# nianticlabs/acezero

Hardware: AMD Instinct MI355X
Metric: ACE patches/sec (higher is better)
Workload: dtype bf16; 1 GPU; 7-Scenes-chess-like ace_zero mapping step: 8M-patch bf16 feature buffer in HBM, batch 5120 per GPU, default head (1 block, 2 103 300 params), tanh loss, 1cyclepoly AdamW, pose_refinement none; buffer_patches=8000000, batch_per_gpu=5120, global_batch=5120, parallelism=dp1

## Files before the change

acezero_amd/_native.py:

```python
import contextlib
import ctypes as C
import os

import torch

from . import build as _build

_lib = None

ACEZ_OK = 0
ERRORS = {-1: "ACEZ_ERR_INVALID", -2: "ACEZ_ERR_HIP", -3: "ACEZ_ERR_NODEVICE", -4: "ACEZ_ERR_NAN"}


class RansacParams(C.Structure):
    _fields_ = [("hypotheses", C.c_int32), ("max_tries", C.c_int32), ("inlier_threshold", C.c_float),
                ("inlier_alpha", C.c_float), ("max_reproj", C.c_float), ("subsampling", C.c_int32),
                ("max_ref_steps", C.c_int32), ("reserved", C.c_int32)]


class Intrinsics(C.Structure):
    _fields_ = [("focal", C.c_float), ("ppx", C.c_float), ("ppy", C.c_float)]


class HeadDesc(C.Structure):
# ... 106 lines not shown
    "acez_trainer_create": (C.c_int, [C.POINTER(C.c_void_p), C.POINTER(TrainConfig), C.POINTER(ParamBuffers), C.c_int]),
    "acez_trainer_destroy": (None, [C.c_void_p]),
    "acez_trainer_set_buffer": (C.c_int, [C.c_void_p, C.POINTER(TrainBuffer)]),
    "acez_trainer_sync_weights": (C.c_int, [C.c_void_p, C.c_void_p]),
    "acez_train_backward": (C.c_int, [C.c_void_p, C.c_void_p, C.c_int, C.c_void_p]),
    "acez_train_update": (C.c_int, [C.c_void_p, C.c_void_p]),
    "acez_train_update_next": (C.c_int, [C.c_void_p, C.c_void_p, C.c_int, C.c_void_p]),
    "acez_train_update_layers": (C.c_int, [C.c_void_p, C.c_int, C.c_int, C.c_void_p]),
    "acez_trainer_export_weights16": (C.c_int, [C.c_void_p, C.c_int, C.c_int, C.c_void_p, C.c_void_p]),
    "acez_trainer_import_weights16": (C.c_int, [C.c_void_p, C.c_int, C.c_int, C.c_void_p, C.c_void_p]),
    "acez_trainer_import_weights16_all": (C.c_int, [C.c_void_p, C.c_int, C.c_int, C.c_void_p, C.c_void_p]),
    "acez_train_step": (C.c_int, [C.c_void_p, C.c_void_p, C.c_int, C.c_void_p]),
    "acez_train_step_next": (C.c_int, [C.c_void_p, C.c_void_p, C.c_int, C.c_void_p, C.c_int, C.c_void_p]),
    "acez_train_group_create": (C.c_int, [C.POINTER(C.c_void_p), C.POINTER(C.c_void_p), C.c_int]),
    "acez_train_group_destroy": (None, [C.c_void_p]),
    "acez_train_group_step": (C.c_int, [C.c_void_p, C.POINTER(C.c_void_p), C.POINTER(C.c_int32), C.POINTER(C.c_void_p),
                                        C.POINTER(C.c_int32), C.c_void_p]),
    "acez_trainer_get_state": (C.c_int, [C.c_void_p, C.POINTER(TrainState), C.c_void_p]),
    "acez_trainer_get_log": (C.c_int, [C.c_void_p, C.c_int, C.c_int, C.c_void_p, C.c_void_p, C.c_void_p]),
    "acez_trainer_last_scene_coords": (C.c_int, [C.c_void_p, C.c_void_p, C.c_int, C.c_void_p]),
    "acez_trainer_set_profiling": (C.c_int, [C.c_void_p, C.c_int]),
    "acez_trainer_get_profile": (C.c_int, [C.c_void_p, C.c_void_p, C.c_void_p]),
    "acez_trainer_seq_status": (C.c_int, [C.c_void_p, C.POINTER(C.c_int), C.POINTER(C.c_int), C.POINTER(C.c_int)]),
    "acez_trainer_debug_read": (C.c_int, [C.c_void_p, C.c_int, C.c_int, C.c_void_p, C.c_int64, C.c_void_p]),
    "acez_trainer_get_poses": (C.c_int, [C.c_void_p, C.c_void_p, C.c_void_p]),
    "acez_head_forward": (C.c_int, [C.c_void_p, C.c_void_p, C.c_int, C.c_void_p, C.c_void_p]),
    "acez_head_forward_maps": (C.c_int, [C.c_void_p, C.c_void_p, C.c_int, C.c_int, C.c_int, C.c_void_p, C.c_void_p]),
    "acez_buffer_warp_views": (C.c_int, [C.c_void_p, C.c_int, C.c_int, C.c_int, C.c_void_p, C.c_void_p, C.c_void_p, C.c_int, C.c_int, C.c_int,
                                        C.c_void_p, C.c_void_p, C.c_int, C.c_int, C.c_void_p, C.c_void_p]),
    "acez_buffer_sample_views": (C.c_int, [C.c_void_p, C.c_void_p, C.c_int, C.c_int, C.c_int, C.c_int, C.c_int, C.c_uint64, C.c_uint64,
                                           C.c_int32, C.c_void_p, C.c_void_p, C.c_void_p, C.c_void_p, C.c_void_p]),
    "acez_buffer_sample_views_table": (C.c_int, [C.c_void_p, C.c_int64, C.c_void_p, C.c_int64, C.c_void_p, C.c_int, C.c_int, C.c_int, C.c_int,
                                                 C.c_uint64, C.c_uint64, C.c_int32, C.c_void_p, C.c_void_p, C.c_void_p, C.c_void_p,
                                                 C.c_void_p]),
    "acez_encoder_create": (C.c_int, [C.POINTER(C.c_void_p), C.POINTER(C.c_void_p), C.POINTER(C.c_void_p), C.c_int, C.c_int, C.c_int,
                                      C.c_int, C.c_int, C.c_int]),
    "acez_encoder_destroy": (None, [C.c_void_p]),
    "acez_encoder_output_size": (C.c_int, [C.c_int, C.c_int, C.POINTER(C.c_int), C.POINTER(C.c_int)]),
    "acez_encoder_forward": (C.c_int, [C.c_void_p, C.c_void_p, C.c_int, C.c_int, C.c_int, C.c_void_p, C.c_void_p]),
    "acez_point_cloud_filter": (C.c_int, [C.c_void_p, C.c_void_p, C.c_void_p, C.c_int, C.c_int, C.c_int, C.c_float, C.c_int, C.c_int,
                                          C.c_int, C.c_uint64, C.c_uint64, C.c_int, C.c_void_p, C.c_void_p, C.c_void_p, C.c_void_p,
                                          C.c_void_p, C.c_void_p]),
    "acez_align_create": (C.c_int, [C.POINTER(C.c_void_p), C.c_int, C.c_int, C.c_int]),
    "acez_align_destroy": (None, [C.c_void_p]),
    "acez_align_evaluate": (C.c_int, [C.c_void_p, C.c_void_p, C.c_void_p, C.c_void_p, C.c_int, C.POINTER(AlignParams), C.c_void_p,
                                      C.c_void_p, C.POINTER(C.c_double), C.POINTER(C.c_int32), C.c_void_p, C.c_void_p, C.c_void_p,
# ... 86 lines not shown
```

acezero_amd/csrc/head_api.hip:

```cpp
#include "head_kernels.hip"
#include "pose_fused.hip"
#include "head_maps.hip"
#include "acez_common.h"
#include "conv_launch.h"
#include <stdlib.h>
#include <string.h>
#include <algorithm>
#include "acez_common.h"
#include <vector>
#include <new>

using namespace acez;

struct StepCarry {
  bool wave_pending = false;
  const int64_t* idx = nullptr;
  int n = 0;
  bool in_alt = false;
  void hold(const int64_t* i, int k, bool alt) { idx = i; n = k; in_alt = alt; }
  void drop_batch() { hold(nullptr, 0, false); }
};

struct acez_trainer {
  char* arena_base = nullptr;
// ... 44 lines not shown
  bool pose_fused = true;
  int pose_tile = 4;
  bool pose_wt_valid = false;
  float* row_dT = nullptr;
  int* row_image = nullptr;
  bool profiling = false;
  std::vector<hipEvent_t> ev_pool;
  struct EvUse { int cls, i0, i1, launches; };
  std::vector<EvUse> ev_used;
  size_t ev_next = 0;
  int prof_launches = 0;
  bool seq = true;
  bool f16 = false;
  int last_nblk = 0;
  int n_cus = 0;
  uint32_t* seq_flags = nullptr;
  uint32_t seq_base[64] = {};
  uint32_t* seq_xcc = nullptr;
  int* seq_err = nullptr;
  uint32_t seq_spin_limit = 40000;
  int seq_faults = 0;
  int seq_probe = -1;
  bool loss_in_chain = true;
  long seq_launches = 0, seq_fault_at = -1;
  bool wgrad_opt = true;
  float* wg_xch = nullptr;
  uint32_t* wg_flags = nullptr;
  uint32_t wg_epoch = 0;
  uint16_t* R0_alt = nullptr;
  int4* batch_meta_alt = nullptr;
  long wgo_fault_at = -1;
  int wgo_fault_mod = 0;
  uint32_t* wg_status = nullptr;
  WgoFaultRec* wg_rec = nullptr;
  int wgo_recovered = 0;
  bool inference_only = false;
  bool sizing = false;
  size_t sized_total = 0;
  unsigned long long* pose_trace = nullptr;
  unsigned long long* wgo_trace = nullptr;
};

enum { KC_SCHED = 0, KC_GATHER, KC_GEMM_FWD, KC_LOSS, KC_GEMM_DGRAD, KC_WGRAD, KC_REDUCE, KC_ADAMW, KC_COUNT };

static int loss_blocks(int n) { return (n + 15) / 16; }
static int gather_blocks(int n) { return (n + 3) / 4 < 1024 ? (n + 3) / 4 : 1024; }
// ... 522 lines not shown
  a.In[f1] = tr->R[tr->nb + 1]; a.In[f2] = tr->out[f1];
  a.slabs = tr->slabs; a.slab_stride = tr->n_wide; a.M = n; a.nslabs = tr->nslabs; a.n_layers = tr->L; a.st = st; a.zeros = tr->zeros;
}


enum class Flow { Fused, Backward, Update };
enum class Opt { None, WgradOpt, AdamwPose, AdamwNext, AdamwSplitPose, Adamw };
enum class NextAt { None, Loss, Optimiser };

struct StepPlan {
  Flow flow;
  bool begin_launch = false, begin_gathers = false, begin_pose = false;
  NextAt next_at = NextAt::None;
  Opt opt = Opt::None;
};

struct StepRun {
  acez_trainer* tr;
  StepPlan plan;
  const int64_t* idx; int n;
  const int64_t* next; int n_next;
  int nblk;
  bool loss_in_chain = false;
  hipStream_t s, ps;
  const TrainState* st;
};

static StepPlan plan_step(const acez_trainer* tr, Flow flow, const int64_t* idx, int n, const int64_t* next, int n_next) {
  StepPlan p{flow};
  const bool pf = tr->pose_fused, announced = next && n_next > 0;
  if (flow != Flow::Update) {
    const StepCarry& c = tr->carry;
    const bool have = !c.in_alt && c.idx == idx && c.n == n;
    p.begin_gathers = !have || (!pf && c.wave_pending);
    p.begin_pose = pf;
    p.begin_launch = p.begin_gathers || pf;
    if (flow == Flow::Backward) return p;
  }
  if (flow == Flow::Fused && wgrad_opt_usable(tr)) p.opt = Opt::WgradOpt;
  else if (flow == Flow::Fused && pf) p.opt = Opt::AdamwPose;
  else if (announced && tr->cfg.pose_refinement == 0 && tr->have_buf) p.opt = Opt::AdamwNext;
  else if (tr->cfg.pose_refinement != 0) p.opt = Opt::AdamwSplitPose;
  else p.opt = Opt::Adamw;
  if (announced && (p.opt == Opt::WgradOpt || p.opt == Opt::AdamwPose)) p.next_at = NextAt::Loss;
  else if (p.opt == Opt::AdamwNext || (announced && p.opt == Opt::AdamwSplitPose && pf && tr->have_buf)) p.next_at = NextAt::Optimiser;
  return p;
// ... 103 lines not shown
    ++tr->prof_launches;
  };
  ProfScope dchain(tr, s, collect ? -1 : KC_GEMM_DGRAD);
  dgrad(f2, f1, nullptr, tr->dZ[f1], nullptr);
  int cur = 0;
  dgrad(f1, 3 * tr->nb + 2, nullptr, tr->dZ[3 * tr->nb + 2], tr->dR[cur]);
  for (int b = tr->nb; b >= 0; --b) {
    dgrad(3 * b + 2, 3 * b + 1, nullptr, tr->dZ[3 * b + 1], nullptr);
    dgrad(3 * b + 1, 3 * b, nullptr, tr->dZ[3 * b], nullptr);
    if (b > 0) {
      dgrad(3 * b, 3 * (b - 1) + 2, tr->dR[cur], tr->dZ[3 * (b - 1) + 2], tr->dR[cur ^ 1]);
      cur ^= 1;
    }
  }
  if (collect) *collect = sq;
  else if (seq && inchain) {
    const SeqLossArgs x = train_loss_in_chain(*inchain);
    launch_rowseq<true>(tr, sq, n, st, s, &x);
  }
  else if (seq) launch_rowseq<true>(tr, sq, n, st, s);
  else if (inchain) abort();
}

static void launch_weight_grads(acez_trainer* tr, const StepPlan& p, int n, int nblk, const TrainState* st, hipStream_t s) {
  const bool fused = p.flow == Flow::Fused;
  const int f2 = 3 * (tr->nb + 1) + 1;
  {
    GradReduceArgs a{};
    a.slabs = tr->slabs; a.slab_stride = tr->n_wide; a.nslabs = tr->nslabs; a.fc3_partials = tr->fc3_partials;
    a.fc3_stride = tr->fc3_stride; a.stat_partials = tr->stat_partials; a.n_loss_blocks = nblk; a.grad = tr->pb.d_grad;
    a.n_wide = tr->n_wide; a.n_params = tr->n_params; a.st = st;
    a.bias_partials = tr->bias_partials; a.bias_layer_stride = tr->bias_layer_stride; a.n_layers = tr->L;
    a.skip_wide = fused ? 1 : 0;
    a.fault = tr->seq_err;
    for (int l = 0; l < tr->L; ++l) a.bias_count[l] = (l == f2) ? nblk : (n + 79) / 80;
    tr->last_reduce = a;
  }
  {
    WgradArgs a{};
    fill_wgrad_args(tr, a, n, st);
    ProfScope ps(tr, s, KC_WGRAD);
    const int groups = tr->L * tr->nslabs;
    if (p.opt == Opt::WgradOpt) {
      WgradOptArgs o{};
      fill_adam_args(tr, o.ad);
      o.ad.tail = tr->last_reduce;
// ... 86 lines not shown
}

static void pose_fwd_launches(acez_trainer* tr, hipStream_t q) {
  if (tr->cfg.pose_refinement == 2) pose_forward(tr, &tr->st->active, q);
  if (tr->cfg.pose_refinement == 1)
    hipLaunchKernelGGL(pose_compose_kernel, dim3((tr->buf.n_images + 255) / 256), dim3(256), 0, q, (const float*)tr->pa1,
                       (const float*)tr->pb.d_pose_params, 1.0f, tr->pose_cur, tr->buf.n_images, (const int*)&tr->st->active, tr->cfg.pose_refinement_ortho);
}
static void pose_bwd_launches(acez_trainer* tr, int n, hipStream_t q) {
  if (tr->cfg.pose_refinement == 0) return;
  const int I = tr->buf.n_images;
  const int* active = &tr->st->active;
  hipLaunchKernelGGL(pose_grad_reduce2_kernel, dim3((I + 15) / 16), dim3(256), 0, q, (const float*)tr->row_dT, (const int*)tr->row_image, n, tr->pdT, I, active);
  if (tr->cfg.pose_refinement == 2) {
    hipLaunchKernelGGL(pose_mlp_bwd_kernel, dim3((I + PN_IMG - 1) / PN_IMG), dim3(256), 0, q, pose_net_args(tr, active));
    launch_pose_wgrad(tr, active, false, q);
  } else {
    hipLaunchKernelGGL(pose_compose_bwd_kernel, dim3((I + 255) / 256), dim3(256), 0, q, (const float*)tr->pa1, (const float*)tr->pb.d_pose_params, 1.0f,
                       (const float*)tr->pdT, tr->pb.d_grad + tr->n_params + 4, I, active, tr->cfg.pose_refinement_ortho);
  }
}

static StepRun start_run(acez_trainer* tr, Flow flow, const int64_t* idx, int n, const int64_t* next, int n_next, hipStream_t s) {
  return StepRun{tr, plan_step(tr, flow, idx, n, next, n_next), idx, n, next, n_next, loss_blocks(n), false, s, tr->pose_stream ? tr->pose_stream : s, nullptr};
}

static void launch_chain(const StepRun& r, bool bwd) {
  if (bwd) launch_dgrad(r.tr, r.n, r.st, r.s, nullptr, r.loss_in_chain ? &r : nullptr);
  else launch_forward(r.tr, r.tr->R[0], r.n, r.st, r.s);
}

template <class Chains>
static int run_steps(StepRun* runs, int count, Chains chains) {
  for (int i = 0; i < count; ++i) {
    StepRun& r = runs[i];
    acez_trainer* tr = r.tr;
    tr->last_n = r.n;
    begin_step(tr, r.plan, r.idx, r.n, r.s);
    r.st = tr->st;
    if (r.ps != r.s) {
      ACEZ_HIP_CHECK(hipEventRecord(tr->ev_begin, r.s));
      ACEZ_HIP_CHECK(hipStreamWaitEvent(r.ps, tr->ev_begin, 0));
    }
    if (!tr->pose_fused) pose_fwd_launches(tr, r.ps);
    if (r.ps != r.s) ACEZ_HIP_CHECK(hipEventRecord(tr->ev_pose_fwd, r.ps));
  }
  chains(false);
  for (int i = 0; i < count; ++i) {
    StepRun& r = runs[i];
    acez_trainer* tr = r.tr;
    if (r.ps != r.s) ACEZ_HIP_CHECK(hipStreamWaitEvent(r.s, tr->ev_pose_fwd, 0));
// ... 9 lines not shown
  for (int i = 0; i < count; ++i) {
    StepRun& r = runs[i];
    acez_trainer* tr = r.tr;
    launch_weight_grads(tr, r.plan, r.n, r.nblk, r.st, r.s);
    if (r.ps != r.s) ACEZ_HIP_CHECK(hipStreamWaitEvent(r.s, tr->ev_pose_bwd, 0));
    if (tr->pose_fused && r.plan.flow == Flow::Backward) launch_pose_wgrad(tr, &tr->st->active, false, r.s);
    ACEZ_HIP_CHECK(hipGetLastError());
    if (r.plan.flow == Flow::Fused) {
      const int rc = launch_update(tr, r.plan, r.s, 0, tr->L, r.next, r.n_next);
      if (rc != ACEZ_OK) return rc;
    }
  }
  return ACEZ_OK;
}

static int train_step_impl(acez_trainer* tr, Flow flow, const int64_t* d_indices, int n, void* stream, const int64_t* d_next = nullptr, int n_next = 0) {
  ACEZ_REQUIRE(tr && d_indices, "null pointer");
  ACEZ_REQUIRE(!tr->inference_only, "an inference-only context (acez_train_config.inference_only) cannot train");
  ACEZ_REQUIRE(tr->have_buf, "acez_trainer_set_buffer has not been called");
  ACEZ_REQUIRE(n > 0 && n <= tr->max_batch, "n must be in [1, max_batch]");
  ACEZ_HIP_CHECK(hipSetDevice(tr->device));
  StepRun r = start_run(tr, flow, d_indices, n, d_next, n_next, (hipStream_t)stream);
  r.loss_in_chain = tr->loss_in_chain && r.plan.opt == Opt::WgradOpt && seq_usable(tr, n);
  return run_steps(&r, 1, [&](bool bwd) { launch_chain(r, bwd); });
}

extern "C" int acez_train_backward(acez_trainer* tr, const int64_t* d_indices, int n, void* stream) {
  return train_step_impl(tr, Flow::Backward, d_indices, n, stream);
}

static int train_update_impl(acez_trainer* tr, void* stream, int layer_lo, int layer_hi, const int64_t* d_next = nullptr, int n_next = 0) {
  ACEZ_REQUIRE(tr, "null trainer");
  ACEZ_REQUIRE(!tr->inference_only, "an inference-only context (acez_train_config.inference_only) cannot train");
  if (layer_hi < 0) layer_hi = tr->L;
  ACEZ_REQUIRE(layer_lo >= 0 && layer_lo <= layer_hi && layer_hi <= tr->L, "layer range out of bounds");
  ACEZ_HIP_CHECK(hipSetDevice(tr->device));
  return launch_update(tr, plan_step(tr, Flow::Update, nullptr, 0, d_next, n_next), (hipStream_t)stream, layer_lo, layer_hi, d_next, n_next);
}

extern "C" int acez_train_update(acez_trainer* tr, void* stream) { return train_update_impl(tr, stream, 0, -1); }
extern "C" int acez_train_update_next(acez_trainer* tr, const int64_t* d_indices_next, int n_next, void* stream) {
  ACEZ_REQUIRE(n_next >= 0 && (!tr || n_next <= tr->max_batch), "n_next must be in [0, max_batch]");
  return train_update_impl(tr, stream, 0, -1, d_indices_next, n_next);
}

extern "C" int acez_train_update_layers(acez_trainer* tr, int layer_lo, int layer_hi, void* stream) {
  return train_update_impl(tr, stream, layer_lo, layer_hi);
// ... 239 lines not shown
```

acezero_amd/csrc/head_kernels.hip:

```cpp
#include <hip/hip_runtime.h>
#include <stdint.h>
#include "head_kernels.h"
#include "gemm_common.h"

namespace acez {


template <int GR = 4>
__device__ __forceinline__ void gather_rows(const uint16_t* __restrict__ feat, const int64_t* __restrict__ idx, uint16_t* __restrict__ out, int n,
                                            int wave, int nwaves, int lane, const GatherMeta& meta) {
  const bool held = meta.hold && *meta.hold;
  for (int r0 = wave; r0 < n; r0 += GR * nwaves) {
    int r[GR];
    bool ok[GR];
    int64_t s[GR];
#pragma unroll
    for (int j = 0; j < GR; ++j) { r[j] = r0 + j * nwaves; ok[j] = r[j] < n; s[j] = idx[ok[j] ? r[j] : r0]; }
    uint4 v[GR];
#pragma unroll
    for (int j = 0; j < GR; ++j) v[j] = *reinterpret_cast<const uint4*>(feat + s[j] * 512 + lane * 8);
    int view[GR];
    float2 tp[GR];
    if (meta.dst) {
#pragma unroll
// ... 390 lines not shown
}

struct SeqLayer {
  const uint16_t *In, *W;
  const float* bias;
  const uint16_t *add, *res;
  uint2* mask_out;
  const uint2* mask_in;
  uint16_t *out_main, *out_aux;
  float* bias_partials;
  int aux_mode, pad;
};
constexpr int SEQ_MAX_LAYERS = 8;
struct RowSeqArgs {
  SeqLayer layer[SEQ_MAX_LAYERS];
  int n_layers, M;
  const TrainState* st;
  uint32_t* flags;
  uint32_t base[64];
  uint32_t spin_limit;
  uint32_t* xcc_dbg;
};

template <bool BWD, class E, int SEAM0>
__device__ __forceinline__ void rowseq_layers(const RowSeqArgs& a, uint16_t* smem, const int mt, const int n0) {
  for (int layer = 0; layer < a.n_layers; ++layer) {
    const SeqLayer& y = a.layer[layer];
    RowGemmArgs g;
    g.In = y.In; g.W = y.W; g.bias = y.bias; g.add = y.add; g.mask_out = y.mask_out; g.mask_in = y.mask_in; g.res = y.res; g.out_main = y.out_main; g.out_aux = y.out_aux;
    g.bias_partials = y.bias_partials; g.M = a.M; g.N = 512; g.K = 512; g.relu = BWD ? 0 : 1; g.aux_mode = y.aux_mode; g.st = a.st;
    g.absmax = (BWD && a.st) ? const_cast<uint32_t*>(a.st->dz_absmax_slots) : nullptr;
    SeqLink q;
    q.flag = a.flags + mt * 32; q.target = (a.base[mt] + (uint32_t)(layer + SEAM0)) * 32u;
    q.first = !SEAM0 && layer == 0; q.wait = SEAM0 || layer > 0; q.signal = layer + 1 < a.n_layers;
    q.next_W = q.signal ? a.layer[layer + 1].W : nullptr;
    q.flag_index = (uint32_t)(mt * 32); q.limit = a.spin_limit;
    if (!BWD) {
      if (y.aux_mode == AUX_RESIDUAL) rowgemm80_body<true, false, false, AUX_RESIDUAL, true, E>(g, smem, 1, mt, n0, q);
      else rowgemm80_body<true, false, false, AUX_NONE, true, E>(g, smem, 1, mt, n0, q);
    } else {
      if (y.add) rowgemm80_body<false, true, true, AUX_UNMASKED, true, E>(g, smem, 1, mt, n0, q);
      else if (y.aux_mode == AUX_UNMASKED) rowgemm80_body<false, false, true, AUX_UNMASKED, true, E>(g, smem, 1, mt, n0, q);
      else rowgemm80_body<false, false, true, AUX_NONE, true, E>(g, smem, 1, mt, n0, q);
    }
  }
}

template <bool BWD, class E = EltBf16>
__global__ __launch_bounds__(512) void rowseq_kernel(RowSeqArgs a) {
  __shared__ __attribute__((aligned(16))) uint16_t smem[RG80_SMEM_SEQ];
  const int mtiles = (a.M + 79) / 80;
  const int per_xcd = (mtiles + 7) >> 3;
  const int jx = blockIdx.x >> 3;
  const int mt = (blockIdx.x & 7) * per_xcd + (jx >> 2);
  if (mt >= mtiles) return;
  if (a.xcc_dbg && threadIdx.x == 0) {
    const uint32_t xcc = __builtin_amdgcn_s_getreg((3 << 11) | 20) & 15u;
    atomicOr(a.xcc_dbg + (blockIdx.x & 7), 1u << xcc);
    a.xcc_dbg[8 + mt * 4 + (jx & 3)] = xcc;
  }
  if ((a.st && !a.st->active) || a.flags[64 * 32]) {
    if (threadIdx.x == 0) {
      const uint32_t inc = 8u * (uint32_t)(a.n_layers - 1);
      asm volatile("global_atomic_add %0, %1, off" ::"v"(a.flags + mt * 32), "v"(inc) : "memory");
    }
    return;
  }
  rowseq_layers<BWD, E, 0>(a, smem, mt, (jx & 3) * 128);
}

__global__ __launch_bounds__(512) void seq_probe_kernel(uint32_t* rec , int mtiles) {
  __shared__ __attribute__((aligned(16))) uint16_t smem[RG80_SMEM_SEQ];
  const int per_xcd = (mtiles + 7) >> 3;
  const int jx = blockIdx.x >> 3;
  const int mt = (blockIdx.x & 7) * per_xcd + (jx >> 2);
  if (threadIdx.x == 0) smem[0] = (uint16_t)blockIdx.x;
  __syncthreads();
  if (mt >= mtiles || threadIdx.x != 0) return;
  const uint32_t xcc = __builtin_amdgcn_s_getreg((3 << 11) | 20) & 15u;
  rec[mt * 4 + (jx & 3)] = (xcc << 16) | smem[0];
}

static inline void launch_rowgemm(const RowGemmArgs& g, hipStream_t s, bool f16 = false) {
  const bool br = g.bias != nullptr;
  const int mtiles = (g.M + 79) / 80;
  const dim3 grid(8 * 4 * ((mtiles + 7) / 8));
#define ACEZ_RG(...)                                                                                               \
  do {                                                                                                             \
    if (f16) hipLaunchKernelGGL((rowgemm80_kernel<__VA_ARGS__, EltF16>), grid, dim3(512), 0, s, g);                \
    else hipLaunchKernelGGL((rowgemm80_kernel<__VA_ARGS__>), grid, dim3(512), 0, s, g);                            \
  } while (0)
// ... 1253 lines not shown
  return -sum;
}

constexpr int WGO_PF = 17;
__device__ __forceinline__ void lds_wait_ge(uint32_t* f, uint32_t target) {
  while (__hip_atomic_load(f, __ATOMIC_RELAXED, __HIP_MEMORY_SCOPE_WORKGROUP) < target) __builtin_amdgcn_s_sleep(1);
  asm volatile("" ::: "memory");
}
__device__ __forceinline__ void lds_bump(uint32_t* f) {
  asm volatile("s_waitcnt lgkmcnt(0)" ::: "memory");
  if ((threadIdx.x & 63) == 0) __hip_atomic_fetch_add(f, 1u, __ATOMIC_RELAXED, __HIP_MEMORY_SCOPE_WORKGROUP);
}

struct SeqLossArgs {
  LossArgs loss;
  int nblk;
  const uint16_t* feat;
  const int64_t* idx_next;
  uint16_t* out_next;
  int n_next;
  GatherMeta meta;
};

template <class E = EltBf16>
__global__ __launch_bounds__(512) void rowseq_loss_kernel(RowSeqArgs a, SeqLossArgs x) {
  __shared__ __attribute__((aligned(16))) uint16_t smem[RG80_SMEM_SEQ];
  const int mtiles = (a.M + 79) / 80;
  const int per_xcd = (mtiles + 7) >> 3;
  const int jx = blockIdx.x >> 3;
  const int mt = (blockIdx.x & 7) * per_xcd + (jx >> 2);
  if (mt >= mtiles) return;
  const int t = threadIdx.x, l = t & 63;
  const int w = __builtin_amdgcn_readfirstlane(t >> 6);
  const int nt = jx & 3, n0 = nt * 128;
  if (a.xcc_dbg && t == 0) {
    const uint32_t xcc = __builtin_amdgcn_s_getreg((3 << 11) | 20) & 15u;
    atomicOr(a.xcc_dbg + (blockIdx.x & 7), 1u << xcc);
    a.xcc_dbg[8 + mt * 4 + nt] = xcc;
  }
  uint32_t* const qsync = reinterpret_cast<uint32_t*>(smem + RG80_SMEM);
  if (t < 2) qsync[t] = 0u;
  asm volatile("s_waitcnt lgkmcnt(0)" ::: "memory");
  __builtin_amdgcn_s_barrier();
  const bool dead = (a.st && !a.st->active) || a.flags[64 * 32];
  if (w >= 4) {
    const int lw = w - 4;
    if (!dead) {
#pragma unroll
      for (int j = 0; j < 4; ++j) {
        const int row = (lw * 4 + j) * 8 + (l >> 3);
        const uint16_t* g = a.layer[0].W + (size_t)(n0 + row) * 512 + ((l & 7) ^ ((row >> 1) & 7)) * 8;
#pragma unroll
        for (int kt = 0; kt < 4; ++kt)
          __builtin_amdgcn_global_load_lds((gvoid_t*)(g + kt * 64), (lvoid_t*)(smem + kt * RG80_STAGE + (lw * 4 + j) * 8 * 64), 16, 0, 0);
      }
    }
    if (nt != 0 && x.n_next > 0) gather_rows<8>(x.feat, x.idx_next, x.out_next, x.n_next, (mt * 3 + nt - 1) * 4 + lw, mtiles * 12, l, x.meta);
  }
  if (dead) {
    if (t == 0) {
      const uint32_t inc = 8u * (uint32_t)a.n_layers;
      asm volatile("global_atomic_add %0, %1, off" ::"v"(a.flags + mt * 32), "v"(inc) : "memory");
    }
    return;
  }
  if (w < 4 || nt == 0) {
    const int quartet = w >> 2;
    const int block = 5 * mt + (nt == 0 ? quartet : nt + 1);
    if (block < x.nblk) {
      float* scratch = reinterpret_cast<float*>(smem + 4 * RG80_STAGE) + quartet * (3 * 4 * 4 * 4);
      uint32_t* const f = qsync + quartet;
      loss_body<false, true, E, 4>(x.loss, block, w & 3, l, nullptr, scratch, LossPre{0, 0, 0, 0.f, 0.f}, [f] { lds_bump(f); lds_wait_ge(f, 4u); });
    }
    ACEZ_VMCNT(0);
    if (l == 0) {
      const uint32_t inc = nt == 0 ? 1u : 2u;
      asm volatile("global_atomic_add %0, %1, off" ::"v"(a.flags + mt * 32), "v"(inc) : "memory");
    }
  }
  rowseq_layers<true, E, 1>(a, smem, mt, n0);
}

#ifdef ACEZ_DIAG
#define WGO_STAMP(i) do { if (o.trace && (threadIdx.x & 63) == 0) o.trace[((size_t)blockIdx.x * 12 + (threadIdx.x >> 6)) * 8 + (i)] = __builtin_amdgcn_s_memtime(); } while (0)
#else
#define WGO_STAMP(i) do { } while (0)
#endif
template <class E = EltBf16>
__global__ __launch_bounds__(WGRAD_THREADS) void wgrad_opt_kernel(WgradArgs a, WgradOptArgs o, PostArgs post) {
  constexpr int RING = WGRAD_RING;
  static_assert(RING >= 3, "two free ring slots are used as staging areas after the K loop");
  __shared__ __attribute__((aligned(16))) uint16_t smem[RING][2][64 * 128];
  __shared__ uint32_t wsync[2];
  const int t = threadIdx.x, l = t & 63;
  const int w = __builtin_amdgcn_readfirstlane(t >> 6);
  const int b = blockIdx.x;
  const int xcd = b & 7, jx = b >> 3;
  const int layer = xcd + 8 * (jx >> 5), slab = (jx >> 4) & 1, tile = jx & 15;
  if (layer >= a.n_layers) return;
  if (t < 2) wsync[t] = 0;
  WGO_STAMP(0);
  const int n0 = (tile >> 2) * 128, c0 = (tile & 3) * 128;
  const AdamArgs& ad = o.ad;
// ... 234 lines not shown
```

acezero_amd/head.py:

```python
import ctypes as C
import math

import numpy as np
import torch

from . import DEFAULT_DTYPE
from . import _native as N

LOSS_TYPES = {"tanh": 0, "dyntanh": 1, "l1": 2, "l1+sqrt": 3, "l1+logl1": 4, "l1+log": 4}
SCHEDULES = {"constant": 0, "1cyclepoly": 1, "circle": 2}
DTYPES = {"bf16": 0, "fp16": 1}


def resolve_dtype(dtype=None):
    import os
    dtype = (dtype or os.environ.get("ACEZ_DTYPE") or DEFAULT_DTYPE).lower()
    if dtype in ("fp32", "float32"):
        raise NotImplementedError("fp32 arithmetic (--use_half False) is not implemented; choose dtype='fp16' (the reference's "
                                  "autocast format) or 'bf16'")
    if dtype not in DTYPES:
        raise ValueError("dtype must be 'bf16' or 'fp16'")
    return dtype


# ... 112 lines not shown
        cfg.max_batch, cfg.global_batch = self.max_batch, self.global_batch
        cfg.loss_type = LOSS_TYPES[loss_type]
        cfg.soft_clamp, cfg.soft_clamp_min, cfg.circle_schedule = soft_clamp, soft_clamp_min, int(circle_schedule)
        cfg.hard_clamp, cfg.depth_min, cfg.depth_max, cfg.depth_target = hard_clamp, depth_min, depth_max, depth_target
        cfg.inlier_px_threshold = inlier_px_threshold
        cfg.schedule, cfg.iterations = SCHEDULES[schedule], int(iterations)
        cfg.lr_min, cfg.lr_max, cfg.warmup_iterations, cfg.warmup_lr = lr_min, lr_max, int(warmup_iterations), warmup_lr
        cfg.cooldown_iterations, cfg.cooldown_trigger_percent = int(cooldown_iterations), cooldown_trigger_percent
        cfg.beta1, cfg.beta2, cfg.eps, cfg.weight_decay = 0.9, 0.999, 1e-8, 1e-2
        cfg.refine_calibration, cfg.focal_init, cfg.calib_lr = int(refine_calibration), float(focal_init), calib_lr
        cfg.pose_refinement = 2 if self.pose_mlp else (1 if self.pose_naive else 0)
        cfg.pose_refinement_wait, cfg.pose_refinement_lr = int(pose_refinement_wait), float(pose_refinement_lr)
        cfg.pose_refinement_weight = float(pose_refinement_weight)
        if refinement_ortho not in ("gram-schmidt", "procrustes"):
            raise ValueError("refinement_ortho must be 'gram-schmidt' or 'procrustes'")
        cfg.pose_refinement_ortho = 1 if refinement_ortho == "procrustes" else 0
        cfg.compute_dtype = DTYPES[self.dtype]
        cfg.inference_only = 1 if inference_only else 0
        pb = N.ParamBuffers(_ptr(self.params), _ptr(self.adam_m), _ptr(self.adam_v), _ptr(self.grad), self.n_params,
                            _ptr(self.pose_params), _ptr(self.pose_m), _ptr(self.pose_v), self.n_pose)
        h = C.c_void_p()
        N.check(self.lib.acez_trainer_create(C.byref(h), C.byref(cfg), C.byref(pb), self.device.index))
        self._h = h
        self._buf = None
        self.iterations = int(iterations)

    def close(self):
        if getattr(self, "_h", None):
            self.lib.acez_trainer_destroy(self._h)
            self._h = None

    def __del__(self):
        try:
            self.close()
        except Exception:
            pass

    def _views(self):
        out, o = {}, 0
        for name in layer_names(self.nb):
            out[name + ".weight"] = self.params[o:o + 262144].view(512, 512, 1, 1)
            o += 262144
            out[name + ".bias"] = self.params[o:o + 512]
            o += 512
        out["fc3.weight"] = self.params[o:o + self.no * 512].view(self.no, 512, 1, 1)
        o += self.no * 512
# ... 91 lines not shown

    def master_tensors(self):
        return [self.params, self.adam_m, self.adam_v]

    def step(self, indices, next_indices=None):
        assert indices.dtype == torch.int64 and indices.is_cuda and indices.is_contiguous()
        if next_indices is None:
            N.check(self.lib.acez_train_step(self._h, _ptr(indices), int(indices.numel()), _stream()))
        else:
            assert next_indices.dtype == torch.int64 and next_indices.is_cuda and next_indices.is_contiguous()
            self._next_keepalive = next_indices
            N.check(self.lib.acez_train_step_next(self._h, _ptr(indices), int(indices.numel()), _ptr(next_indices), int(next_indices.numel()),
                                                  _stream()))

    def state(self):
        st = N.TrainState()
        rc = self.lib.acez_trainer_get_state(self._h, C.byref(st), _stream())
        if rc not in (0, -4):
            N.check(rc)
        return {"iteration": st.iteration, "max_iterations": st.max_iterations, "in_cooldown": bool(st.in_cooldown),
                "nan": bool(st.nan_flag), "lr": st.lr, "loss": st.last_loss, "batch_inliers": st.last_batch_inliers,
                "focal_scale": st.focal_scale, "grad_scale": st.grad_scale, "opt_steps": st.opt_steps}

    def seq_status(self):
        en, pr, fl = C.c_int(0), C.c_int(0), C.c_int(0)
        N.check(self.lib.acez_trainer_seq_status(self._h, C.byref(en), C.byref(pr), C.byref(fl)))
        return {"enabled": bool(en.value), "probe": pr.value, "faults": fl.value}

    def log(self, first, count):
        loss = np.zeros(count, np.float32)
        inl = np.zeros(count, np.float32)
        N.check(self.lib.acez_trainer_get_log(self._h, first, count, loss.ctypes.data_as(C.c_void_p),
                                              inl.ctypes.data_as(C.c_void_p), _stream()))
        return loss, inl

    def last_scene_coords(self, n):
        out = np.zeros((n, 3), np.float32)
        N.check(self.lib.acez_trainer_last_scene_coords(self._h, out.ctypes.data_as(C.c_void_p), n, _stream()))
        return out

    KERNEL_CLASSES = ("sched", "gather", "gemm_fwd", "loss", "gemm_dgrad", "wgrad", "grad_reduce", "adamw")

    def set_profiling(self, on):
        N.check(self.lib.acez_trainer_set_profiling(self._h, int(bool(on))))

    def get_profile(self):
        ms = np.zeros(8, np.float32)
        cnt = np.zeros(8, np.int32)
        N.check(self.lib.acez_trainer_get_profile(self._h, ms.ctypes.data_as(C.c_void_p), cnt.ctypes.data_as(C.c_void_p)))
        return {k: (float(ms[i]), int(cnt[i])) for i, k in enumerate(self.KERNEL_CLASSES)}
# ... 82 lines not shown
```

include/acez.h:

```cpp
#ifndef ACEZ_H
#define ACEZ_H

#include <stdint.h>

#ifdef __cplusplus
extern "C" {
#endif

#define ACEZ_OK 0
#define ACEZ_ERR_INVALID (-1)
#define ACEZ_ERR_HIP (-2)
#define ACEZ_ERR_NODEVICE (-3)
#define ACEZ_ERR_NAN (-4)

const char* acez_last_error(void);
const char* acez_version(void);
int acez_device_count(void);


typedef struct acez_ransac_params {
  int32_t hypotheses;
  int32_t max_tries;
  float inlier_threshold;
  float inlier_alpha;
// ... 184 lines not shown
int acez_train_update_next(acez_trainer* tr, const int64_t* d_indices_next, int n_next, void* stream);
int acez_train_update_layers(acez_trainer* tr, int layer_lo, int layer_hi, void* stream);
int acez_trainer_export_weights16(acez_trainer* tr, int layer_lo, int layer_hi, void* d_dst, void* stream);
int acez_trainer_import_weights16(acez_trainer* tr, int layer_lo, int layer_hi, const void* d_src, void* stream);
int acez_trainer_import_weights16_all(acez_trainer* tr, int own_lo, int own_hi, const void* d_src_all, void* stream);

int acez_train_step(acez_trainer* tr, const int64_t* d_indices, int n, void* stream);
int acez_train_step_next(acez_trainer* tr, const int64_t* d_indices, int n, const int64_t* d_indices_next, int n_next, void* stream);

typedef struct acez_train_group acez_train_group;
int acez_train_group_create(acez_train_group** out, acez_trainer* const* members, int h);
void acez_train_group_destroy(acez_train_group* g);
int acez_train_group_step(acez_train_group* g, const int64_t* const* d_indices, const int32_t* n, const int64_t* const* d_next,
                          const int32_t* n_next, void* stream);

int acez_trainer_get_state(acez_trainer* tr, acez_train_state* h_out, void* stream);
int acez_trainer_get_log(acez_trainer* tr, int first, int count, float* h_loss, float* h_inliers, void* stream);
int acez_trainer_last_scene_coords(acez_trainer* tr, float* h_xyz, int n, void* stream);

int acez_trainer_set_profiling(acez_trainer* tr, int enable);
int acez_trainer_get_profile(acez_trainer* tr, float* h_ms8, int32_t* h_counts8);

int acez_trainer_seq_status(acez_trainer* tr, int* enabled, int* probe, int* faults);

int acez_trainer_debug_read(acez_trainer* tr, int kind, int index, void* h_out, int64_t bytes, void* stream);

int acez_trainer_get_poses(acez_trainer* tr, float* h_poses34, void* stream);

int acez_head_forward(acez_trainer* tr, const void* d_features, int n, float* d_out_xyz, void* stream);

int acez_head_forward_maps(acez_trainer* tr, const void* d_features, int n_frames, int h, int w, float* d_out_maps,
                           void* stream);

#define ACEZ_ENCODER_LAYERS 11

typedef struct acez_encoder acez_encoder;

int acez_encoder_create(acez_encoder** out, const float* const* h_weights, const float* const* h_biases,
                        int out_channels, int max_frames, int max_h, int max_w, int compute_dtype, int device);
void acez_encoder_destroy(acez_encoder* enc);

int acez_encoder_output_size(int h, int w, int* out_h, int* out_w);

int acez_encoder_forward(acez_encoder* enc, const float* d_images, int n_frames, int h, int w, void* d_features,
                         void* stream);

// ... 121 lines not shown
```

Baseline: 37.80 million patches/s.

## Fuse forward, loss and dgrad chain into one persistent rowstep kernel

Result: faster. 38.96 million patches/s (median of 6 runs) (+3.1%).

```diff
diff --git a/acezero_amd/_native.py b/acezero_amd/_native.py
--- a/acezero_amd/_native.py
+++ b/acezero_amd/_native.py
@@ -152,6 +152,8 @@
     "acez_trainer_set_profiling": (C.c_int, [C.c_void_p, C.c_int]),
     "acez_trainer_get_profile": (C.c_int, [C.c_void_p, C.c_void_p, C.c_void_p]),
     "acez_trainer_seq_status": (C.c_int, [C.c_void_p, C.POINTER(C.c_int), C.POINTER(C.c_int), C.POINTER(C.c_int)]),
+    "acez_trainer_step_chain_status": (C.c_int, [C.c_void_p, C.POINTER(C.c_int), C.POINTER(C.c_longlong)]),
+    "acez_trainer_set_step_chain": (C.c_int, [C.c_void_p, C.c_int]),
     "acez_trainer_debug_read": (C.c_int, [C.c_void_p, C.c_int, C.c_int, C.c_void_p, C.c_int64, C.c_void_p]),
     "acez_trainer_get_poses": (C.c_int, [C.c_void_p, C.c_void_p, C.c_void_p]),
     "acez_head_forward": (C.c_int, [C.c_void_p, C.c_void_p, C.c_int, C.c_void_p, C.c_void_p]),
diff --git a/acezero_amd/csrc/head_api.hip b/acezero_amd/csrc/head_api.hip
--- a/acezero_amd/csrc/head_api.hip
+++ b/acezero_amd/csrc/head_api.hip
@@ -90,6 +90,8 @@
   int seq_faults = 0;
   int seq_probe = -1;
   bool loss_in_chain = true;
+  bool step_chain = true;
+  long step_chain_steps = 0;
   long seq_launches = 0, seq_fault_at = -1;
   bool wgrad_opt = true;
   float* wg_xch = nullptr;
@@ -658,6 +660,7 @@
   const int64_t* next; int n_next;
   int nblk;
   bool loss_in_chain = false;
+  bool step_chain = false;
   hipStream_t s, ps;
   const TrainState* st;
 };
@@ -807,6 +810,30 @@
   else if (inchain) abort();
 }
 
+static void launch_rowstep(const StepRun& r) {
+  acez_trainer* tr = r.tr;
+  std::vector<SeqLayer> fwd, bwd;
+  launch_forward(tr, tr->R[0], r.n, r.st, r.s, &fwd);
+  launch_dgrad(tr, r.n, r.st, r.s, &bwd);
+  if (fwd.size() > SEQ_MAX_LAYERS || bwd.size() > SEQ_MAX_LAYERS || bwd.empty()) abort();
+  const int mtiles = (r.n + 79) / 80;
+  RowStepArgs a{};
+  for (size_t i = 0; i < fwd.size(); ++i) a.fwd[i] = fwd[i];
+  for (size_t i = 0; i < bwd.size(); ++i) a.bwd[i] = bwd[i];
+  a.n_fwd = (int)fwd.size(); a.n_bwd = (int)bwd.size(); a.M = r.n;
+  a.st = r.st ? r.st : tr->st_infer; a.flags = tr->seq_flags; a.xcc_dbg = tr->seq_xcc; a.spin_limit = tr->seq_spin_limit;
+  for (int mt = 0; mt < 64; ++mt) a.base[mt] = tr->seq_base[mt];
+  if (tr->seq_fault_at >= tr->seq_launches && tr->seq_fault_at < tr->seq_launches + 2)
+    for (int mt = 0; mt < 64; ++mt) a.base[mt] += 1u << 20;
+  tr->seq_launches += 2;
+  a.x = train_loss_in_chain(r);
+  if (tr->f16) hipLaunchKernelGGL(rowstep_kernel<EltF16>, dim3(32 * ((mtiles + 7) / 8)), dim3(512), 0, r.s, a);
+  else hipLaunchKernelGGL(rowstep_kernel<EltBf16>, dim3(32 * ((mtiles + 7) / 8)), dim3(512), 0, r.s, a);
+  for (int mt = 0; mt < mtiles; ++mt) tr->seq_base[mt] += (uint32_t)(a.n_fwd + a.n_bwd);
+  tr->prof_launches += a.n_fwd + a.n_bwd;
+  ++tr->step_chain_steps;
+}
+
 static void launch_weight_grads(acez_trainer* tr, const StepPlan& p, int n, int nblk, const TrainState* st, hipStream_t s) {
   const bool fused = p.flow == Flow::Fused;
   const int f2 = 3 * (tr->nb + 1) + 1;
@@ -939,11 +966,14 @@
 }
 
 static StepRun start_run(acez_trainer* tr, Flow flow, const int64_t* idx, int n, const int64_t* next, int n_next, hipStream_t s) {
-  return StepRun{tr, plan_step(tr, flow, idx, n, next, n_next), idx, n, next, n_next, loss_blocks(n), false, s, tr->pose_stream ? tr->pose_stream : s, nullptr};
+  return StepRun{tr, plan_step(tr, flow, idx, n, next, n_next), idx, n, next, n_next, loss_blocks(n), false, false, s, tr->pose_stream ? tr->pose_stream : s, nullptr};
 }
 
 static void launch_chain(const StepRun& r, bool bwd) {
-  if (bwd) launch_dgrad(r.tr, r.n, r.st, r.s, nullptr, r.loss_in_chain ? &r : nullptr);
+  if (r.step_chain) {
+    if (bwd) launch_rowstep(r);
+  }
+  else if (bwd) launch_dgrad(r.tr, r.n, r.st, r.s, nullptr, r.loss_in_chain ? &r : nullptr);
   else launch_forward(r.tr, r.tr->R[0], r.n, r.st, r.s);
 }
 
@@ -999,7 +1029,21 @@
   ACEZ_HIP_CHECK(hipSetDevice(tr->device));
   StepRun r = start_run(tr, flow, d_indices, n, d_next, n_next, (hipStream_t)stream);
   r.loss_in_chain = tr->loss_in_chain && r.plan.opt == Opt::WgradOpt && seq_usable(tr, n);
+  r.step_chain = r.loss_in_chain && tr->step_chain && !tr->profiling && tr->L <= SEQ_MAX_LAYERS;
   return run_steps(&r, 1, [&](bool bwd) { launch_chain(r, bwd); });
+}
+
+extern "C" int acez_trainer_set_step_chain(acez_trainer* tr, int enable) {
+  ACEZ_REQUIRE(tr, "null trainer");
+  tr->step_chain = enable != 0;
+  return ACEZ_OK;
+}
+
+extern "C" int acez_trainer_step_chain_status(acez_trainer* tr, int* enabled, long long* steps) {
+  ACEZ_REQUIRE(tr, "null trainer");
+  if (enabled) *enabled = (tr->step_chain && tr->loss_in_chain && wgrad_opt_usable(tr) && tr->L <= SEQ_MAX_LAYERS) ? 1 : 0;
+  if (steps) *steps = tr->step_chain_steps;
+  return ACEZ_OK;
 }
 
 extern "C" int acez_train_backward(acez_trainer* tr, const int64_t* d_indices, int n, void* stream) {
diff --git a/acezero_amd/csrc/head_kernels.hip b/acezero_amd/csrc/head_kernels.hip
--- a/acezero_amd/csrc/head_kernels.hip
+++ b/acezero_amd/csrc/head_kernels.hip
@@ -436,19 +436,28 @@
   uint32_t* xcc_dbg;
 };
 
-template <bool BWD, class E, int SEAM0>
-__device__ __forceinline__ void rowseq_layers(const RowSeqArgs& a, uint16_t* smem, const int mt, const int n0) {
-  for (int layer = 0; layer < a.n_layers; ++layer) {
-    const SeqLayer& y = a.layer[layer];
+struct SeqCtx {
+  int M;
+  const TrainState* st;
+  uint32_t* flags;
+  uint32_t base;
+  uint32_t seam0;
+  uint32_t limit;
+};
+
+template <bool BWD, class E, bool HEAD, bool TAIL = false>
+__device__ __forceinline__ void rowseq_layers(const SeqLayer* layers, const int n_layers, const SeqCtx& c, uint16_t* smem, const int mt, const int n0) {
+  for (int layer = 0; layer < n_layers; ++layer) {
+    const SeqLayer& y = layers[layer];
     RowGemmArgs g;
     g.In = y.In; g.W = y.W; g.bias = y.bias; g.add = y.add; g.mask_out = y.mask_out; g.mask_in = y.mask_in; g.res = y.res; g.out_main = y.out_main; g.out_aux = y.out_aux;
-    g.bias_partials = y.bias_partials; g.M = a.M; g.N = 512; g.K = 512; g.relu = BWD ? 0 : 1; g.aux_mode = y.aux_mode; g.st = a.st;
-    g.absmax = (BWD && a.st) ? const_cast<uint32_t*>(a.st->dz_absmax_slots) : nullptr;
+    g.bias_partials = y.bias_partials; g.M = c.M; g.N = 512; g.K = 512; g.relu = BWD ? 0 : 1; g.aux_mode = y.aux_mode; g.st = c.st;
+    g.absmax = (BWD && c.st) ? const_cast<uint32_t*>(c.st->dz_absmax_slots) : nullptr;
     SeqLink q;
-    q.flag = a.flags + mt * 32; q.target = (a.base[mt] + (uint32_t)(layer + SEAM0)) * 32u;
-    q.first = !SEAM0 && layer == 0; q.wait = SEAM0 || layer > 0; q.signal = layer + 1 < a.n_layers;
-    q.next_W = q.signal ? a.layer[layer + 1].W : nullptr;
-    q.flag_index = (uint32_t)(mt * 32); q.limit = a.spin_limit;
+    q.flag = c.flags + mt * 32; q.target = (c.base + c.seam0 + (uint32_t)layer) * 32u;
+    q.first = !HEAD && layer == 0; q.wait = HEAD || layer > 0; q.signal = TAIL || layer + 1 < n_layers;
+    q.next_W = layer + 1 < n_layers ? layers[layer + 1].W : nullptr;
+    q.flag_index = (uint32_t)(mt * 32); q.limit = c.limit;
     if (!BWD) {
       if (y.aux_mode == AUX_RESIDUAL) rowgemm80_body<true, false, false, AUX_RESIDUAL, true, E>(g, smem, 1, mt, n0, q);
       else rowgemm80_body<true, false, false, AUX_NONE, true, E>(g, smem, 1, mt, n0, q);
@@ -480,7 +489,7 @@
     }
     return;
   }
-  rowseq_layers<BWD, E, 0>(a, smem, mt, (jx & 3) * 128);
+  rowseq_layers<BWD, E, false>(a.layer, a.n_layers, SeqCtx{a.M, a.st, a.flags, a.base[mt], 0u, a.spin_limit}, smem, mt, (jx & 3) * 128);
 }
 
 __global__ __launch_bounds__(512) void seq_probe_kernel(uint32_t* rec , int mtiles) {
@@ -1780,6 +1789,76 @@
   GatherMeta meta;
 };
 
+__device__ __forceinline__ bool seq_poll_expired(const uint32_t* flag, uint32_t target, uint32_t limit) {
+  uint32_t vseen, sseen, spins, timed;
+  asm volatile(
+      "s_mov_b32 %[spins], 0\n\t"
+      "s_mov_b32 %[timed], 0\n"
+      "1:\n\t"
+      "global_load_dword %[vseen], %[flag], off sc1\n\t"
+      "s_waitcnt vmcnt(0)\n\t"
+      "v_readfirstlane_b32 %[sseen], %[vseen]\n\t"
+      "s_sub_i32 %[sseen], %[sseen], %[target]\n\t"
+      "s_cmp_ge_i32 %[sseen], 0\n\t"
+      "s_cbranch_scc1 2f\n\t"
+      "s_sleep 1\n\t"
+      "s_add_u32 %[spins], %[spins], 1\n\t"
+      "s_cmp_lt_u32 %[spins], %[limit]\n\t"
+      "s_cbranch_scc1 1b\n\t"
+      "s_mov_b32 %[timed], 1\n"
+      "2:"
+      : [vseen] "=&v"(vseen), [sseen] "=&s"(sseen), [spins] "=&s"(spins), [timed] "=&s"(timed)
+      : [flag] "v"(flag), [target] "s"(target), [limit] "s"(limit)
+      : "memory", "scc");
+  return timed != 0;
+}
+
+template <class E, bool FWD_SEAM>
+__device__ __forceinline__ void rowseq_loss_stage(const uint16_t* W0, const SeqLossArgs& x, const SeqCtx& c, const bool dead, uint16_t* smem,
+                                                  const int mt, const int nt, const int mtiles) {
+  const int t = threadIdx.x, l = t & 63;
+  const int w = __builtin_amdgcn_readfirstlane(t >> 6);
+  const int n0 = nt * 128;
+  uint32_t* const qsync = reinterpret_cast<uint32_t*>(smem + RG80_SMEM);
+  if (t < 2) qsync[t] = 0u;
+  asm volatile("s_waitcnt lgkmcnt(0)" ::: "memory");
+  __builtin_amdgcn_s_barrier();
+  if (w >= 4) {
+    const int lw = w - 4;
+    if (!dead) {
+#pragma unroll
+      for (int j = 0; j < 4; ++j) {
+        const int row = (lw * 4 + j) * 8 + (l >> 3);
+        const uint16_t* g = W0 + (size_t)(n0 + row) * 512 + ((l & 7) ^ ((row >> 1) & 7)) * 8;
+#pragma unroll
+        for (int kt = 0; kt < 4; ++kt)
+          __builtin_amdgcn_global_load_lds((gvoid_t*)(g + kt * 64), (lvoid_t*)(smem + kt * RG80_STAGE + (lw * 4 + j) * 8 * 64), 16, 0, 0);
+      }
+    }
+    if (nt != 0 && x.n_next > 0) gather_rows<8>(x.feat, x.idx_next, x.out_next, x.n_next, (mt * 3 + nt - 1) * 4 + lw, mtiles * 12, l, x.meta);
+  }
+  if (dead) return;
+  if (w < 4 || nt == 0) {
+    uint32_t* const flag = c.flags + mt * 32;
+    const int quartet = w >> 2;
+    const int block = 5 * mt + (nt == 0 ? quartet : nt + 1);
+    if (FWD_SEAM && seq_poll_expired(flag, (c.base + c.seam0 - 1u) * 32u, c.limit) && l == 0) {
+      __hip_atomic_store(c.flags + 64 * 32, 1u, __ATOMIC_RELAXED, __HIP_MEMORY_SCOPE_AGENT);
+      if (c.st) __hip_atomic_store(const_cast<int*>(&c.st->active), 0, __ATOMIC_RELAXED, __HIP_MEMORY_SCOPE_AGENT);
+    }
+    if (block < x.nblk) {
+      float* scratch = reinterpret_cast<float*>(smem + 4 * RG80_STAGE) + quartet * (3 * 4 * 4 * 4);
+      uint32_t* const f = qsync + quartet;
+      loss_body<false, true, E, 4>(x.loss, block, w & 3, l, nullptr, scratch, LossPre{0, 0, 0, 0.f, 0.f}, [f] { lds_bump(f); lds_wait_ge(f, 4u); });
+    }
+    ACEZ_VMCNT(0);
+    if (l == 0) {
+      const uint32_t inc = nt == 0 ? 1u : 2u;
+      asm volatile("global_atomic_add %0, %1, off" ::"v"(flag), "v"(inc) : "memory");
+    }
+  }
+}
+
 template <class E = EltBf16>
 __global__ __launch_bounds__(512) void rowseq_loss_kernel(RowSeqArgs a, SeqLossArgs x) {
   __shared__ __attribute__((aligned(16))) uint16_t smem[RG80_SMEM_SEQ];
@@ -1788,55 +1867,64 @@
   const int jx = blockIdx.x >> 3;
   const int mt = (blockIdx.x & 7) * per_xcd + (jx >> 2);
   if (mt >= mtiles) return;
-  const int t = threadIdx.x, l = t & 63;
-  const int w = __builtin_amdgcn_readfirstlane(t >> 6);
-  const int nt = jx & 3, n0 = nt * 128;
-  if (a.xcc_dbg && t == 0) {
+  const int nt = jx & 3;
+  if (a.xcc_dbg && threadIdx.x == 0) {
     const uint32_t xcc = __builtin_amdgcn_s_getreg((3 << 11) | 20) & 15u;
     atomicOr(a.xcc_dbg + (blockIdx.x & 7), 1u << xcc);
     a.xcc_dbg[8 + mt * 4 + nt] = xcc;
   }
-  uint32_t* const qsync = reinterpret_cast<uint32_t*>(smem + RG80_SMEM);
-  if (t < 2) qsync[t] = 0u;
-  asm volatile("s_waitcnt lgkmcnt(0)" ::: "memory");
-  __builtin_amdgcn_s_barrier();
   const bool dead = (a.st && !a.st->active) || a.flags[64 * 32];
-  if (w >= 4) {
-    const int lw = w - 4;
-    if (!dead) {
-#pragma unroll
-      for (int j = 0; j < 4; ++j) {
-        const int row = (lw * 4 + j) * 8 + (l >> 3);
-        const uint16_t* g = a.layer[0].W + (size_t)(n0 + row) * 512 + ((l & 7) ^ ((row >> 1) & 7)) * 8;
-#pragma unroll
-        for (int kt = 0; kt < 4; ++kt)
-          __builtin_amdgcn_global_load_lds((gvoid_t*)(g + kt * 64), (lvoid_t*)(smem + kt * RG80_STAGE + (lw * 4 + j) * 8 * 64), 16, 0, 0);
-      }
-    }
-    if (nt != 0 && x.n_next > 0) gather_rows<8>(x.feat, x.idx_next, x.out_next, x.n_next, (mt * 3 + nt - 1) * 4 + lw, mtiles * 12, l, x.meta);
-  }
+  const SeqCtx c{a.M, a.st, a.flags, a.base[mt], 1u, a.spin_limit};
+  rowseq_loss_stage<E, false>(a.layer[0].W, x, c, dead, smem, mt, nt, mtiles);
   if (dead) {
-    if (t == 0) {
+    if (threadIdx.x == 0) {
       const uint32_t inc = 8u * (uint32_t)a.n_layers;
       asm volatile("global_atomic_add %0, %1, off" ::"v"(a.flags + mt * 32), "v"(inc) : "memory");
     }
     return;
   }
-  if (w < 4 || nt == 0) {
-    const int quartet = w >> 2;
-    const int block = 5 * mt + (nt == 0 ? quartet : nt + 1);
-    if (block < x.nblk) {
-      float* scratch = reinterpret_cast<float*>(smem + 4 * RG80_STAGE) + quartet * (3 * 4 * 4 * 4);
-      uint32_t* const f = qsync + quartet;
-      loss_body<false, true, E, 4>(x.loss, block, w & 3, l, nullptr, scratch, LossPre{0, 0, 0, 0.f, 0.f}, [f] { lds_bump(f); lds_wait_ge(f, 4u); });
-    }
-    ACEZ_VMCNT(0);
-    if (l == 0) {
-      const uint32_t inc = nt == 0 ? 1u : 2u;
+  rowseq_layers<true, E, true>(a.layer, a.n_layers, c, smem, mt, nt * 128);
+}
+
+struct RowStepArgs {
+  SeqLayer fwd[SEQ_MAX_LAYERS], bwd[SEQ_MAX_LAYERS];
+  int n_fwd, n_bwd, M;
+  const TrainState* st;
+  uint32_t* flags;
+  uint32_t base[64];
+  uint32_t spin_limit;
+  uint32_t* xcc_dbg;
+  SeqLossArgs x;
+};
+static_assert(sizeof(RowStepArgs) <= 4096, "kernel-argument segment");
+
+template <class E = EltBf16>
+__global__ __launch_bounds__(512) void rowstep_kernel(RowStepArgs a) {
+  __shared__ __attribute__((aligned(16))) uint16_t smem[RG80_SMEM_SEQ];
+  const int mtiles = (a.M + 79) / 80;
+  const int per_xcd = (mtiles + 7) >> 3;
+  const int jx = blockIdx.x >> 3;
+  const int mt = (blockIdx.x & 7) * per_xcd + (jx >> 2);
+  if (mt >= mtiles) return;
+  const int nt = jx & 3;
+  if (a.xcc_dbg && threadIdx.x == 0) {
+    const uint32_t xcc = __builtin_amdgcn_s_getreg((3 << 11) | 20) & 15u;
+    atomicOr(a.xcc_dbg + (blockIdx.x & 7), 1u << xcc);
+    a.xcc_dbg[8 + mt * 4 + nt] = xcc;
+  }
+  const bool dead = (a.st && !a.st->active) || a.flags[64 * 32];
+  const uint32_t base = a.base[mt];
+  if (!dead) rowseq_layers<false, E, false, true>(a.fwd, a.n_fwd, SeqCtx{a.M, a.st, a.flags, base, 0u, a.spin_limit}, smem, mt, nt * 128);
+  const SeqCtx c{a.M, a.st, a.flags, base, (uint32_t)a.n_fwd + 1u, a.spin_limit};
+  rowseq_loss_stage<E, true>(a.bwd[0].W, a.x, c, dead, smem, mt, nt, mtiles);
+  if (dead) {
+    if (threadIdx.x == 0) {
+      const uint32_t inc = 8u * (uint32_t)(a.n_fwd + a.n_bwd);
       asm volatile("global_atomic_add %0, %1, off" ::"v"(a.flags + mt * 32), "v"(inc) : "memory");
     }
-  }
-  rowseq_layers<true, E, 1>(a, smem, mt, n0);
+    return;
+  }
+  rowseq_layers<true, E, true>(a.bwd, a.n_bwd, c, smem, mt, nt * 128);
 }
 
 #ifdef ACEZ_DIAG
diff --git a/acezero_amd/head.py b/acezero_amd/head.py
--- a/acezero_amd/head.py
+++ b/acezero_amd/head.py
@@ -1,5 +1,6 @@
 import ctypes as C
 import math
+import os
 
 import numpy as np
 import torch
@@ -158,6 +159,8 @@
         h = C.c_void_p()
         N.check(self.lib.acez_trainer_create(C.byref(h), C.byref(cfg), C.byref(pb), self.device.index))
         self._h = h
+        if os.environ.get("ACEZ_STEP_CHAIN") is not None and hasattr(self.lib, "acez_trainer_set_step_chain"):
+            N.check(self.lib.acez_trainer_set_step_chain(h, int(os.environ["ACEZ_STEP_CHAIN"] != "0")))
         self._buf = None
         self.iterations = int(iterations)
 
@@ -295,10 +298,15 @@
                 "nan": bool(st.nan_flag), "lr": st.lr, "loss": st.last_loss, "batch_inliers": st.last_batch_inliers,
                 "focal_scale": st.focal_scale, "grad_scale": st.grad_scale, "opt_steps": st.opt_steps}
 
-    def seq_status(self):
+    def seq_status(self, step_chain=False):
         en, pr, fl = C.c_int(0), C.c_int(0), C.c_int(0)
         N.check(self.lib.acez_trainer_seq_status(self._h, C.byref(en), C.byref(pr), C.byref(fl)))
-        return {"enabled": bool(en.value), "probe": pr.value, "faults": fl.value}
+        out = {"enabled": bool(en.value), "probe": pr.value, "faults": fl.value}
+        if step_chain:
+            on, steps = C.c_int(0), C.c_longlong(0)
+            N.check(self.lib.acez_trainer_step_chain_status(self._h, C.byref(on), C.byref(steps)))
+            out.update(step_chain=bool(on.value), step_chain_steps=steps.value)
+        return out
 
     def log(self, first, count):
         loss = np.zeros(count, np.float32)
diff --git a/include/acez.h b/include/acez.h
--- a/include/acez.h
+++ b/include/acez.h
@@ -230,6 +230,8 @@
 int acez_trainer_get_profile(acez_trainer* tr, float* h_ms8, int32_t* h_counts8);
 
 int acez_trainer_seq_status(acez_trainer* tr, int* enabled, int* probe, int* faults);
+int acez_trainer_step_chain_status(acez_trainer* tr, int* enabled, long long* steps);
+int acez_trainer_set_step_chain(acez_trainer* tr, int enable);
 
 int acez_trainer_debug_read(acez_trainer* tr, int kind, int index, void* h_out, int64_t bytes, void* stream);
 
```
